# yuhang1008/WildGS-SLAM-Blackwell

Measured on AMD Instinct MI355X. Metric: rasterised Gaussians/s fwd+bwd @1M pts 1080p; PSNR vs ref, higher is better.
Workload: dtype f32; 1 GPU; configs[2]: 1000000 Gaussians, 1920x1080, SH3, single-view fwd+bwd, pose grad on; gaussians=1000000, image=1920x1080, sh_degree=3, num_rendered=13015374, parallelism=dp1 (keyframe views), dp_exchange=none

## Files before the change

wildgs-slam-blackwell_amd/csrc/capi.hip:

```cpp
#include <cstdarg>
#include <cstdio>
#include <cstdlib>
#include <cstring>
#include <vector>

#include <immintrin.h>

#include "wgsr.h"
#include "wgsr_common.h"
#include "wgsr_internal.h"

namespace wgsr {

namespace {
thread_local char g_err[1024] = "";

struct HostCounters {
  uint32_t* buf = nullptr;
  hipEvent_t ev = nullptr;
  hipStream_t side = nullptr;
  hipEvent_t pre = nullptr;
  uint4* mbox = nullptr;
  uint32_t seq = 0;
};
constexpr int kMaxDevices = 64;
int device_slot() {
  int dev = 0;
  return hipGetDevice(&dev) == hipSuccess && dev >= 0 && dev < kMaxDevices ? dev : -1;
}
struct BinningGuess {
  int P = -1, W = 0, H = 0, bshift = -1;
  size_t bytes = 0;
};
BinningGuess& binning_guess() {
  thread_local BinningGuess g[kMaxDevices];
  const int dev = device_slot();
  return g[dev < 0 ? 0 : dev];
}

bool publish_counts() {
  static const bool on = [] {
    const char* e = getenv("WGSR_PUBLISH_COUNTS");
    return !(e && e[0] == '0');
  }();
  return on;
}

HostCounters& host_counters() {
  thread_local HostCounters per_dev[kMaxDevices];
  const int dev = device_slot();
  HostCounters& hc = per_dev[dev < 0 ? 0 : dev];
  if (!hc.buf) {
    void* p = nullptr;
    if (hipHostMalloc(&p, kCounterBytes, hipHostMallocDefault) != hipSuccess) p = nullptr;
    hc.buf = static_cast<uint32_t*>(p);
    if (hipEventCreateWithFlags(&hc.ev, hipEventDisableTiming) != hipSuccess) hc.ev = nullptr;
    if (hipStreamCreateWithFlags(&hc.side, hipStreamNonBlocking) != hipSuccess) hc.side = nullptr;
    if (hc.side && hipEventCreateWithFlags(&hc.pre, hipEventDisableTiming) != hipSuccess) hc.pre = nullptr;
    if (!hc.pre) hc.side = nullptr;
    void* m = nullptr;
    if (publish_counts() &&
        hipHostMalloc(&m, 256, hipHostMallocCoherent | hipHostMallocMapped) == hipSuccess) {
      hc.mbox = static_cast<uint4*>(m);
      *hc.mbox = make_uint4(0u, 0u, 0u, 0u);
    }
  }
  return hc;
}

struct DevCounters {
  uint32_t* buf = nullptr;
  int parity = 0;
  bool failed = false;
};
DevCounters* dev_counters(hipStream_t s) {
  thread_local DevCounters per_dev[kMaxDevices];
  const int dev = device_slot();
// ... 174 lines not shown
  BinLayout BL;
  size_t lists_bytes, bds_bytes, total;
  BinningPlan(size_t N_rect, size_t N_bin, int bshift, bool bin_depth)
      : BL(N_rect), lists_bytes(bshift ? align256(4 * (N_bin << (2 * bshift))) : 0),
        bds_bytes(bin_depth ? align256(16 * N_bin) : 0), total(BL.total + lists_bytes + bds_bytes) {}
};

struct Counts {
  size_t N_rect, N, N_bin;
  uint32_t flags;
  bool published;
};

int start_counts_readback(const Fwd& f, bool bin_depth, HostCounters& hc, PublishJob* pub) {
  if (!hc.buf || !hc.ev) return set_error(WGSR_EHIP, "pinned counter buffer / event allocation failed");
  if (bin_depth && hc.mbox) {
    *pub = PublishJob{f.counter, hc.mbox, hc.seq = (hc.seq % 0xFFFFFFu) + 1u};
  } else if (hc.side && !bin_depth) {
    HIPCHK(hipEventRecord(hc.pre, f.s));
    HIPCHK(hipStreamWaitEvent(hc.side, hc.pre, 0));
    HIPCHK(hipMemcpyAsync(hc.buf, f.counter, kCounterBytes, hipMemcpyDeviceToHost, hc.side));
    HIPCHK(hipEventRecord(hc.ev, hc.side));
  } else {
    HIPCHK(hipMemcpyAsync(hc.buf, f.counter, kCounterBytes, hipMemcpyDeviceToHost, f.s));
    HIPCHK(hipEventRecord(hc.ev, f.s));
  }
  return WGSR_OK;
}

int wait_counts(const Fwd& f, HostCounters& hc, const PublishJob& pub, Counts* c) {
  if (!pub.counter) {
    HIPCHK(hipEventSynchronize(hc.ev));
  } else {
    uint4 rec = make_uint4(0u, 0u, 0u, 0u);
    auto poll = [&]() {
      asm volatile("" ::: "memory");
      const __m128i v = _mm_load_si128(reinterpret_cast<const __m128i*>(const_cast<const uint4*>(hc.mbox)));
      _mm_storeu_si128(reinterpret_cast<__m128i*>(&rec), v);
      return (rec.x >> 8) == pub.seq;
    };
    uint32_t polls = 0;
    while (!poll()) {
      _mm_pause();
      if ((++polls & 1023u) == 0) {
        const hipError_t q = hipStreamQuery(f.s);
        if (q == hipErrorNotReady) continue;
        HIPCHK(q);
        bool seen = false;
        for (int k = 0; k < (1 << 16) && !(seen = poll()); ++k) _mm_pause();
        if (seen) break;
        hc.mbox = nullptr;
        break;
      }
    }
    if (hc.mbox && !(rec.x & 0x80u)) {
      *c = Counts{rec.y, rec.z, rec.w, rec.x & 0x7Fu, true};
      return WGSR_OK;
    }
    HIPCHK(hipMemcpyAsync(hc.buf, f.counter, kCounterBytes, hipMemcpyDeviceToHost, f.s));
    HIPCHK(hipStreamSynchronize(f.s));
  }
  *c = Counts{0, 0, 0, hc.buf[1], false};
  const uint64_t* partial = reinterpret_cast<const uint64_t*>(hc.buf + 4);
  for (int i = 0; i < kRectPairLanes; ++i) {
    c->N_rect += partial[i];
    c->N += partial[kRectPairLanes + i];
    c->N_bin += partial[2 * kRectPairLanes + i];
  }
  return WGSR_OK;
}

int read_depth_range(const Fwd& f, HostCounters& hc, const Counts& c, uint32_t* hi, uint32_t* nlo) {
  if (c.published) {
    HIPCHK(hipMemcpyAsync(hc.buf, f.counter, kCounterBytes, hipMemcpyDeviceToHost, f.s));
    HIPCHK(hipStreamSynchronize(f.s));
  }
  const uint32_t* rw = hc.buf + kDepthRangeOffset / 4;
  *hi = *nlo = 0;
  for (int i = 0; i < kRectPairLanes; ++i) {
    *hi = rw[i] > *hi ? rw[i] : *hi;
    *nlo = rw[kRectPairLanes + i] > *nlo ? rw[kRectPairLanes + i] : *nlo;
  }
  return WGSR_OK;
}

ZeroJob preprocess_zero_job(const Fwd& f, const DevCounters* dc, DepthSched sched) {
  const size_t P = (size_t)f.a.P;
  ZeroJob zj{};
  auto add = [&](void* p, size_t words) {
    if (words) { zj.p[zj.count] = static_cast<float*>(p); zj.n[zj.count++] = words; }
  };
  if (dc) add(dc->buf + (size_t)(dc->parity ^ 1) * (kCounterBytes / 4), kCounterBytes / 4);
  size_t sup_off = depth_sort_sup_offset_words(P);
  const size_t sup_words = sched == DepthSched::kFull     ? sort_sup_words(P, 0, kDepthBits, &sup_off)
                           : sched == DepthSched::kGlobal ? depth_sort_sup_words(P)
                                                          : 0;
  add(f.g<uint32_t>(f.GL.hist) + sup_off, sup_words);
// ... 6 lines not shown
  const size_t P = (size_t)f.a.P;
  uint32_t *dkey = f.g<uint32_t>(GL.dkey), *dkey_alt = f.g<uint32_t>(GL.dkey_alt), *dval = f.g<uint32_t>(GL.dval),
           *dval_alt = f.g<uint32_t>(GL.dval_alt), *hist = f.g<uint32_t>(GL.hist);
  StageTimer T(kStDepthSort, f.s);
  if (full) {
    const bool sup_zeroed = sort_sup_words(P, 0, kDepthBits, nullptr) != 0;
    bool in_alt = false;
    STAGE(f.a, f.s, radix_sort_pairs(dkey, dkey_alt, dval, dval_alt, true, P, 0, kDepthBits, hist,
                                     f.g<uint32_t>(GL.totals), f.s, &in_alt, nullptr, nullptr, sup_zeroed));
    if (in_alt != kFullDepthInAlt) return set_error(WGSR_EHIP, "internal: depth sort parity");
    *depth_order = kFullDepthInAlt ? dval_alt : dval;
    return WGSR_OK;
  }
  if (zero_sup)
    HIPCHK(hipMemsetAsync(hist + depth_sort_sup_offset_words(P), 0, 4 * depth_sort_sup_words(P), f.s));
  STAGE(f.a, f.s, launch_depth_sort(dkey, dkey_alt, dval, dval_alt, P, f.counter + kDepthRangeOffset / 4,
                                    f.counter + 2, hist, f.s));
  *depth_order = dval_alt;
  return WGSR_OK;
}

int queue_scan(const Fwd& f, const uint32_t* depth_order, const PublishJob& pj) {
  const GeomLayout& GL = f.GL;
  StageTimer T(kStOffsetsScan, f.s);
  if (f.bshift) {
    STAGE(f.a, f.s, packed_scan_blocks(f.g<uint32_t>(GL.tb), 1, depth_order, (size_t)f.a.P, f.g<uint32_t>(GL.bsum),
                                       f.s, f.g<uint2>(GL.bsup), pj));
  } else {
    STAGE(f.a, f.s, exclusive_scan_gather(&f.g<ListRec>(GL.lrec)->w.w, depth_order, (size_t)f.a.P,
                                          f.g<uint32_t>(GL.offs), f.g<uint32_t>(GL.slot_start),
                                          f.g<uint32_t>(GL.bsum), f.g<uint32_t>(GL.counter), f.s,
// ... 150 lines not shown
  }
  Fwd f{a, s, Grid(a), GeomLayout((size_t)a.P), ImageLayout(a.W, a.H), bin_shift(a), out_color, out_depth, out_opacity,
        n_touched};
  if (int e = f.alloc(geom_alloc, image_alloc, ctx)) return e;
  DevCounters* dc = dev_counters(s);
  f.counter = dc ? dc->buf + (size_t)dc->parity * (kCounterBytes / 4) : at<uint32_t>(f.geom, f.GL.counter);
  if (!dc) HIPCHK(hipMemsetAsync(f.counter, 0, kCounterBytes, s));
  const DepthSched sched = depth_schedule(f.bshift);
  struct SyncOnError {
    hipStream_t s;
    bool armed = false;
    ~SyncOnError() { if (armed) (void)hipStreamSynchronize(s); }
  } sync_on_error{s};
  { StageTimer T(kStPreprocess, s);
  const hipError_t pe = launch_preprocess(a, f.geom, radii, n_touched, f.counter + 1,
                                          reinterpret_cast<unsigned long long*>(f.counter + 4), f.bshift,
                                          preprocess_zero_job(f, dc, sched), s, f.im<uint32_t>(f.IL.meta));
  if (pe == hipSuccess && dc) dc->parity ^= 1;
  sync_on_error.armed = true;
  STAGE(a, s, pe); }

  HostCounters& hc = host_counters();
  PublishJob pub{};
  if (int e = start_counts_readback(f, sched == DepthSched::kBins, hc, &pub)) return e;
  const uint32_t* depth_order = nullptr;
  if (sched != DepthSched::kBins)
    if (int e = queue_depth_sort(f, sched == DepthSched::kFull, false, &depth_order)) return e;
  if (int e = queue_scan(f, depth_order, pub)) return e;
  BinningGuess& bg = binning_guess();
  void* binning = nullptr;
  size_t binning_have = 0;
  if (bg.P == a.P && bg.W == a.W && bg.H == a.H && bg.bshift == f.bshift && bg.bytes > 0) {
    binning_have = bg.bytes + bg.bytes / 16;
    binning = call_alloc(binning_alloc, ctx, binning_have);
    if (!binning) binning_have = 0;
  }
  Counts c;
  if (int e = wait_counts(f, hc, pub, &c)) return e;
  sync_on_error.armed = false;

  const bool bins_too_full = sched == DepthSched::kBins &&
                             c.N_bin > bin_depth_max_avg() * (size_t)Bins(f.grid.gx, f.grid.gy, f.bshift).n;
  if (bins_too_full) {
// ... 66 lines not shown
  if (!f.bshift || depth_schedule(f.bshift) != DepthSched::kBins)
    return set_error(WGSR_EINVAL, "capacity mode needs sort bins with the per-bin depth sort");
  if (!((size_t)8 << sort_bits(Bins(f.grid.gx, f.grid.gy, f.bshift).n) <= (size_t)16 * f.grid.nt))
    return set_error(WGSR_EINVAL, "capacity mode: the bin bounds do not fit the tile_m region");
  if (int e = f.alloc(geom_alloc, image_alloc, ctx)) return e;
  const size_t C = (size_t)cap;
  const BinningPlan plan(C, C, f.bshift, true);
  void* binning = call_alloc(binning_alloc, ctx, plan.total);
  if (!binning) return set_error(WGSR_EALLOC, "binning buffer allocation failed");
  f.counter = at<uint32_t>(f.geom, f.GL.counter);
  uint32_t* meta = at<uint32_t>(f.image, f.IL.meta);
  HIPCHK(launch_zero_u32(f.counter, kCounterBytes / 4, s));
  const ZeroJob zj = preprocess_zero_job(f, nullptr, DepthSched::kBins);
  { StageTimer T(kStPreprocess, s);
  STAGE(a, s, launch_preprocess(a, f.geom, radii, n_touched, f.counter + 1,
                                reinterpret_cast<unsigned long long*>(f.counter + 4), f.bshift, zj, s, meta)); }
  STAGE(a, s, launch_cap_counts(reinterpret_cast<const unsigned long long*>(f.counter + 4), (uint64_t)C, (uint64_t)C,
                                counts, meta, s));
  if (int e = queue_scan(f, nullptr, PublishJob{})) return e;
  g_depth_order_off = -1;
  return queue_lists_and_render(f, binning, plan, nullptr, true, C, counts + 4);
}

}

namespace wgsr {
namespace {
int render_backward_pairs(const wgsr_raster_args& a, const void* geom, void* binning, void* image,
                          int64_t num_rendered, const float* dL_dcolor, const float* dL_ddepth,
                          wgsr_alloc_fn scratch_alloc, void* ctx, const ZeroJob& zero, hipStream_t s,
                          float4** partial_out, uint8_t** pflag_out) {
  if (!geom || !image || (num_rendered > 0 && !binning))
    return set_error(WGSR_EINVAL, "missing forward state buffers");
  const Grid grid(a);
// ... 150 lines not shown
```

wildgs-slam-blackwell_amd/csrc/raster_pre.hip:

```cpp
#include <algorithm>

#include "raster_sh.h"
#include "wgsr_common.h"
#include "wgsr_internal.h"

namespace wgsr {

namespace {

__device__ __forceinline__ f3 sh_to_rgb(int deg, const float* sh, f3 dir, uint32_t& clamp_bits) {
#pragma clang fp contract(off)
  auto term = [](float c, const float* v) -> f3 { return {c * v[0], c * v[1], c * v[2]}; };
  auto plus = [](f3 a, f3 b) -> f3 { return {a.x + b.x, a.y + b.y, a.z + b.z}; };
  auto minus = [](f3 a, f3 b) -> f3 { return {a.x - b.x, a.y - b.y, a.z - b.z}; };
  f3 r = term(SH_C0, sh);
  if (deg > 0) {
    const float x = dir.x, y = dir.y, z = dir.z;
    r = minus(plus(minus(r, term(SH_C1 * y, sh + 3)), term(SH_C1 * z, sh + 6)), term(SH_C1 * x, sh + 9));
    if (deg > 1) {
      const float xx = x * x, yy = y * y, zz = z * z, xy = x * y, yz = y * z, xz = x * z;
      r = plus(r, term(SH_C2[0] * xy, sh + 12));
      r = plus(r, term(SH_C2[1] * yz, sh + 15));
      r = plus(r, term(SH_C2[2] * (2.f * zz - xx - yy), sh + 18));
      r = plus(r, term(SH_C2[3] * xz, sh + 21));
// ... 89 lines not shown
      tab.y |= len << (8 * (k - 4));
      tab.w |= (uint32_t)(xa - x0) << (8 * (k - 4));
    }
    cnt += len;
  }
  lrec[i].tab = tab;
  if (!finish) clamped[i] = 0u;
  const uint32_t nb = cnt == 0 ? 0u
                               : (uint32_t)((((x1 - 1) >> bshift) - (x0 >> bshift) + 1) *
                                            (((y1 - 1) >> bshift) - (y0 >> bshift) + 1));
  w = make_uint4((uint32_t)r, cnt, cnt | (nb << 16), __float_as_uint(pv.z));
  return make_uint3((uint32_t)((x1 - x0) * (y1 - y0)), cnt, nb);
}

__device__ __forceinline__ void wave_pair_counts(const uint3 ac, uint32_t khi, uint32_t knlo,
                                                 unsigned long long* __restrict__ rect_pairs,
                                                 unsigned long long* __restrict__ list_pairs,
                                                 unsigned long long* __restrict__ bin_pairs,
                                                 uint32_t* __restrict__ drange) {
  const uint32_t slot = blockIdx.x % kRectPairLanes;
  unsigned long long area, cnt, nbin;
  if (wave_any(ac.x >= (1u << 26))) {
    area = ac.x;
    cnt = ac.y;
    nbin = ac.z;
#pragma unroll
    for (int off = 32; off >= 1; off >>= 1) {
      area += __shfl_xor(area, off, 64);
      cnt += __shfl_xor(cnt, off, 64);
      nbin += __shfl_xor(nbin, off, 64);
    }
  } else {
    area = wave_total_u32(ac.x);
    cnt = wave_total_u32(ac.y);
    nbin = wave_total_u32(ac.z);
  }
  const uint32_t kh = wave_maximum_u32(khi), kn = wave_maximum_u32(knlo);
  if (threadIdx.x % 64 == 0) {
    atomicAdd(&rect_pairs[slot], area);
    atomicAdd(&list_pairs[slot], cnt);
    atomicAdd(&bin_pairs[slot], nbin);
    if (kh) atomicMax(&drange[slot], kh);
    if (kn) atomicMax(&drange[kRectPairLanes + slot], kn);
  }
}

constexpr int kPreWave = 64;

template <int kD, int kCh>
__device__ __forceinline__ f3 sh_rgb_lds(const float* __restrict__ s_sh, int lane, f3 dir, uint32_t& cbits) {
  constexpr int K = (kD + 1) * (kD + 1), NF = 3 * K, NCH = (NF + kCh - 1) / kCh;
  float sh[NCH * kCh];
#pragma unroll
  for (int k = 0; k < NCH; ++k) {
    if constexpr (kCh >= 4) {
      const float4 v = reinterpret_cast<const float4*>(s_sh)[k * 64 + lane];
      sh[4 * k] = v.x;
      sh[4 * k + 1] = v.y;
// ... 3 lines not shown
      sh[k] = s_sh[k * 64 + lane];
    }
  }
  return sh_to_rgb(kD, sh, dir, cbits);
}

template <int kCh, int kD>
__global__ __launch_bounds__(kPreWave) void k_preprocess2(
    int P, int D, int M, const float* __restrict__ means, const float* __restrict__ scales,
    const float* __restrict__ rots, const float* __restrict__ opac, const float* __restrict__ shs,
    const float* __restrict__ colors, const float* __restrict__ cov_pre, float scale_mod,
    const float* __restrict__ viewm, const float* __restrict__ projm, const float* __restrict__ campos_p, int W,
    int H, float tanx, float tany, int gx, int gy, int prefiltered, float4* __restrict__ splat,
    ListRec* __restrict__ lrec, uint32_t* __restrict__ clamped,
    uint32_t* __restrict__ dkey, int32_t* __restrict__ radii, int32_t* __restrict__ n_touched,
    uint32_t* __restrict__ err_flag, unsigned long long* __restrict__ rect_pairs,
    unsigned long long* __restrict__ list_pairs, unsigned long long* __restrict__ bin_pairs, int bshift,
    uint32_t* __restrict__ tb, uint8_t* __restrict__ gflag, uint32_t* __restrict__ drange, const ZeroJob zero,
    uint32_t* __restrict__ meta) {
  extern __shared__ float s_sh[];
  const int lane = threadIdx.x;
  const int i0 = blockIdx.x * kPreWave, i = i0 + lane;
  constexpr bool sh_on = kD >= 0;
  const int ic = min(i, P - 1);
  const int ir = cov_pre ? 0 : ic;
  const float* __restrict__ sp = cov_pre ? cov_pre : scales;
  const float* __restrict__ rp = cov_pre ? cov_pre : rots;
  const f3 pl = mk3(means[3 * ic], means[3 * ic + 1], means[3 * ic + 2]);
  const f3 sl = mk3(sp[3 * ir], sp[3 * ir + 1], sp[3 * ir + 2]);
  const float4 ql = make_float4(rp[4 * ir], rp[4 * ir + 1], rp[4 * ir + 2], rp[4 * ir + 3]);
  const float ol = opac[ic];
  asm volatile("" ::"v"(pl.x), "v"(pl.y), "v"(pl.z), "v"(sl.x), "v"(sl.y), "v"(sl.z), "v"(ql.x), "v"(ql.y),
               "v"(ql.z), "v"(ql.w), "v"(ol));
  auto load_slab = [&]() {
// ... 38 lines not shown
    __builtin_amdgcn_s_waitcnt(0);
    __syncthreads();
    if (i < P && w.x != 0u) {
#pragma clang fp contract(off)
      f3 dir = sub3(p, mk3(campos_p[0], campos_p[1], campos_p[2]));
      const float len = sqrtf(dot3(dir, dir));
      dir = mk3(dir.x / len, dir.y / len, dir.z / len);
      uint32_t cbits = 0;
      const f3 rgb = sh_rgb_lds<(kD < 0 ? 0 : kD), kCh>(s_sh, lane, dir, cbits);
      splat[3 * (size_t)i + 0] = ab[0];
      splat[3 * (size_t)i + 1] = ab[1];
      splat[3 * (size_t)i + 2] = make_float4(rgb.x, rgb.y, rgb.z, __uint_as_float(w.w));
      clamped[i] = cbits;
    }
  }
  wave_pair_counts(ac, khi, knlo, rect_pairs, list_pairs, bin_pairs, drange);
  zero_share(zero, blockIdx.x, gridDim.x, lane, kPreWave);
  if (blockIdx.x == 0 && lane == 0) {
    meta[1] = 0u;
    meta[2] = 0u;
  }
}

__global__ __launch_bounds__(256) void k_mark_visible(int P, const float* __restrict__ means,
                                                      const float* __restrict__ viewm, uint8_t* __restrict__ present) {
  const int i = blockIdx.x * blockDim.x + threadIdx.x;
  if (i >= P) return;
  const f3 p = mk3(means[3 * i], means[3 * i + 1], means[3 * i + 2]);
  const f3 pv = xform43(viewm, p);
  present[i] = pv.z > kNearZ ? 1 : 0;
}

}


__global__ __launch_bounds__(64) void k_cap_counts(const unsigned long long* __restrict__ partial,
                                                   uint64_t cap_rect, uint64_t cap_bin, uint32_t* __restrict__ counts,
                                                   uint32_t* __restrict__ meta) {
  const int t = threadIdx.x;
  unsigned long long r = partial[t], e = partial[kRectPairLanes + t], b = partial[2 * kRectPairLanes + t];
#pragma unroll
  for (int off = 32; off >= 1; off >>= 1) {
    r += __shfl_xor(r, off, 64);
    e += __shfl_xor(e, off, 64);
    b += __shfl_xor(b, off, 64);
  }
  if (t == 0) {
    const uint32_t ovf = (r > cap_rect || b > cap_bin) ? 1u : 0u;
    counts[0] = (uint32_t)min(r, 0xFFFFFFFFull);
    counts[1] = (uint32_t)min(e, 0xFFFFFFFFull);
    counts[2] = (uint32_t)min(b, 0xFFFFFFFFull);
    counts[3] = ovf;
    counts[4] = (uint32_t)min(b, (unsigned long long)cap_bin);
    meta[1] = ovf;
  }
}
static_assert(kRectPairLanes == 64, "k_cap_counts: one lane per partial");

hipError_t launch_cap_counts(const unsigned long long* partial, uint64_t cap_rect, uint64_t cap_bin, uint32_t* counts,
                             uint32_t* meta, hipStream_t s) {
  hipLaunchKernelGGL(k_cap_counts, dim3(1), dim3(64), 0, s, partial, cap_rect, cap_bin, counts, meta);
  return hipGetLastError();
}

hipError_t launch_preprocess(const wgsr_raster_args& a, void* geom, int32_t* radii, int32_t* n_touched,
                             uint32_t* err_flag, unsigned long long* rect_pairs, int bshift, const ZeroJob& zero,
                             hipStream_t s, uint32_t* meta) {
  unsigned long long* list_pairs = rect_pairs + kRectPairLanes;
  unsigned long long* bin_pairs = rect_pairs + 2 * kRectPairLanes;
  uint32_t* drange = reinterpret_cast<uint32_t*>(rect_pairs + 3 * kRectPairLanes);
  if (a.P == 0) return hipSuccess;
  const GeomLayout L(a.P);
  const int gx = (a.W + kTile - 1) / kTile, gy = (a.H + kTile - 1) / kTile;
  const bool sh_on = a.shs && !a.colors;
  const bool ch4 = sh_on && (a.M * 3) % 4 == 0 && (reinterpret_cast<uintptr_t>(a.shs) & 15) == 0;
  const int nf = 3 * (a.D + 1) * (a.D + 1);
  const int kch = ch4 ? 4 : 1;
  const size_t lds2 = sh_on ? sizeof(float) * 64 * (size_t)(((nf + kch - 1) / kch) * kch) : 0;
  using PreKernel = decltype(&k_preprocess2<1, -1>);
  static constexpr PreKernel kPre[2][4] = {{k_preprocess2<1, 0>, k_preprocess2<1, 1>, k_preprocess2<1, 2>,
                                            k_preprocess2<1, 3>},
                                           {k_preprocess2<4, 0>, k_preprocess2<4, 1>, k_preprocess2<4, 2>,
                                            k_preprocess2<4, 3>}};
  const PreKernel kern = sh_on ? kPre[ch4 ? 1 : 0][std::min(std::max(a.D, 0), 3)] : k_preprocess2<1, -1>;
  hipLaunchKernelGGL(kern, dim3((a.P + kPreWave - 1) / kPreWave), dim3(kPreWave),
                     lds2, s, a.P, a.D, a.M, a.means3D, a.scales, a.rotations, a.opacities, a.shs, a.colors,
                     a.cov3D_precomp, a.scale_modifier, a.viewmatrix, a.projmatrix, a.campos, a.W, a.H, a.tan_fovx,
                     a.tan_fovy, gx, gy, a.prefiltered, at<float4>(geom, L.splat), at<ListRec>(geom, L.lrec),
                     at<uint32_t>(geom, L.clamped), at<uint32_t>(geom, L.dkey), radii, n_touched, err_flag, rect_pairs,
                     list_pairs, bin_pairs, bshift, at<uint32_t>(geom, L.tb), at<uint8_t>(geom, L.gflag), drange, zero,
                     meta);
  return hipGetLastError();
}

hipError_t launch_mark_visible(int P, const float* means3D, const float* view, uint8_t* present, hipStream_t s) {
  if (P == 0) return hipSuccess;
  hipLaunchKernelGGL(k_mark_visible, dim3((P + 255) / 256), dim3(256), 0, s, P, means3D, view, present);
  return hipGetLastError();
}

}
```

wildgs-slam-blackwell_amd/csrc/sort.hip:

```cpp
#include <stdlib.h>
#include <string.h>

#include "wgsr_common.h"
#include "wgsr_internal.h"

namespace wgsr {

namespace {

__device__ __forceinline__ uint32_t block_excl_scan256(uint32_t v, uint32_t* s_tmp4, uint32_t* total) {
  const int t = threadIdx.x, w = t >> 6, lane = t & 63;
  uint32_t inc = wave_incl_scan(v);
  if (lane == 63) s_tmp4[w] = inc;
  __syncthreads();
  uint32_t base = 0, tot = 0;
#pragma unroll
  for (int i = 0; i < 4; ++i) {
    uint32_t x = s_tmp4[i];
    base += (i < w) ? x : 0u;
    tot += x;
  }
  __syncthreads();
  if (total) *total = tot;
  return base + inc - v;
// ... 332 lines not shown
  __syncthreads();
  const uint32_t cnt = (size_t)n > blk0 ? (uint32_t)min((size_t)kT, (size_t)n - blk0) : 0u;
#pragma unroll
  for (int r = 0; r < K; ++r) {
    const uint32_t i = (uint32_t)t + (uint32_t)NT * r;
    if (i < cnt) {
      const uint2 kv = s_buf[i];
      const uint32_t d = (kv.x >> shift) & mask;
      const uint32_t dst = s_gbase[d] + (i - s_lbase[d]);
      kout[dst] = kv.x;
      vout[dst] = kv.y;
    }
  }
}

static_assert(kRectPairLanes == 64, "one range word per lane");
__device__ __forceinline__ int bitlen32(uint32_t x) {
  return x ? 32 - __clz((int)x) : 0;
}
__device__ __forceinline__ uint32_t wave_max_u32_uniform(uint32_t x) {
  x = max(x, (uint32_t)__builtin_amdgcn_update_dpp(0, (int)x, 0xB1, 0xf, 0xf, true));
  x = max(x, (uint32_t)__builtin_amdgcn_update_dpp(0, (int)x, 0x4E, 0xf, 0xf, true));
  x = max(x, (uint32_t)__builtin_amdgcn_update_dpp(0, (int)x, 0x114, 0xf, 0xf, true));
  x = max(x, (uint32_t)__builtin_amdgcn_update_dpp(0, (int)x, 0x118, 0xf, 0xf, true));
  const uint32_t a = (uint32_t)__builtin_amdgcn_readlane((int)x, 15), b = (uint32_t)__builtin_amdgcn_readlane((int)x, 31);
  const uint32_t c = (uint32_t)__builtin_amdgcn_readlane((int)x, 47), d = (uint32_t)__builtin_amdgcn_readlane((int)x, 63);
  return max(max(a, b), max(c, d));
}
__device__ __forceinline__ uint2 depth_range_reduce(const uint32_t* __restrict__ range) {
  const int lane = threadIdx.x & 63;
  return make_uint2(wave_max_u32_uniform(range[lane]), wave_max_u32_uniform(range[kRectPairLanes + lane]));
}
__device__ __forceinline__ DepthKeyPlan depth_plan_from2(const uint32_t* __restrict__ range2) {
  return depth_key_plan(range2[0], ~range2[1]);
}

template <int I, int PASS>
__global__ __launch_bounds__(256) void k_depth_hist(const uint32_t* __restrict__ keys, uint32_t n,
                                                    const uint32_t* __restrict__ range, uint32_t* __restrict__ range2,
                                                    uint32_t* __restrict__ hist, uint32_t* __restrict__ sup) {
  __shared__ uint32_t s_h[kDepthMaxDigits];
  const int t = threadIdx.x;
  uint32_t k[I];
  const int nv = load_run<I>(keys, n, (size_t)blockIdx.x * (256 * I) + (size_t)t * I, k);
#pragma unroll
  for (int q = 0; q < kDepthMaxDigits / 256; ++q) s_h[t + 256 * q] = 0;
  DepthKeyPlan pl;
  if (PASS == 0) {
    const uint2 r = depth_range_reduce(range);
    if (blockIdx.x == 0 && t == 0) {
      range2[0] = r.x;
      range2[1] = r.y;
    }
    pl = depth_key_plan(r.x, ~r.y);
// ... 365 lines not shown
                                              totals, stream, result_in_alt, digit_bounds, bounds_done, sup_zeroed,
                                              ndev, wide_threads);
    case kSmallSortItems:
      return radix_sort_tiled<kSmallSortItems>(keys, keys_alt, vals, vals_alt, vals_iota, n, begin_bit, end_bit,
                                               status, totals, stream, result_in_alt, digit_bounds, bounds_done,
                                               sup_zeroed, ndev, wide_threads);
    default:
      return radix_sort_tiled<kSortItems>(keys, keys_alt, vals, vals_alt, vals_iota, n, begin_bit, end_bit, status,
                                          totals, stream, result_in_alt, digit_bounds, bounds_done, sup_zeroed,
                                          ndev, wide_threads);
  }
}

template <int I>
static hipError_t depth_sort_tiled(uint32_t* keys, uint32_t* keys_alt, uint32_t* vals, uint32_t* vals_alt, size_t n,
                                   const uint32_t* range, uint32_t* range2, uint32_t* scratch, hipStream_t s) {
  const uint32_t nb = (uint32_t)((n + 256 * I - 1) / (256 * I)), nsup = (nb + kSupBlocks - 1) / kSupBlocks;
  uint32_t* hist = scratch;
  uint32_t* sup = scratch + depth_sort_sup_offset_words(n);
  const size_t sup_pass = (size_t)kDepthMaxDigits * nsup;
  const uint32_t un = (uint32_t)n;
  hipLaunchKernelGGL((k_depth_hist<I, 0>), dim3(nb), dim3(256), 0, s, keys, un, range, range2, hist, sup);
  hipLaunchKernelGGL((k_depth_scatter<I, 0>), dim3(nb), dim3(256), 0, s, keys, vals, un, range2, hist, sup, nsup,
                     keys_alt, vals_alt);
  hipLaunchKernelGGL((k_depth_hist<I, 1>), dim3(nb), dim3(256), 0, s, keys_alt, un, range, range2, hist,
                     sup + sup_pass);
  hipLaunchKernelGGL((k_depth_scatter<I, 1>), dim3(nb), dim3(256), 0, s, keys_alt, vals_alt, un, range2, hist,
                     sup + sup_pass, nsup, keys, vals);
  hipLaunchKernelGGL((k_depth_hist<I, 2>), dim3(nb), dim3(256), 0, s, keys, un, range, range2, hist,
                     sup + 2 * sup_pass);
  hipLaunchKernelGGL((k_depth_scatter<I, 2>), dim3(nb), dim3(256), 0, s, keys, vals, un, range2, hist,
                     sup + 2 * sup_pass, nsup, keys_alt, vals_alt);
  return hipGetLastError();
}

hipError_t launch_depth_sort(uint32_t* keys, uint32_t* keys_alt, uint32_t* vals, uint32_t* vals_alt, size_t n,
                             const uint32_t* range, uint32_t* range2, uint32_t* scratch, hipStream_t s) {
  if (n == 0) return hipSuccess;
  if (n > (size_t)kStCount) return hipErrorInvalidValue;
  switch (sort_items(n)) {
    case kTinySortItems:
      return depth_sort_tiled<kTinySortItems>(keys, keys_alt, vals, vals_alt, n, range, range2, scratch, s);
    case kSmallSortItems:
      return depth_sort_tiled<kSmallSortItems>(keys, keys_alt, vals, vals_alt, n, range, range2, scratch, s);
    default:
      return depth_sort_tiled<kSortItems>(keys, keys_alt, vals, vals_alt, n, range, range2, scratch, s);
  }
}

hipError_t exclusive_scan_gather(const uint32_t* vals, const uint32_t* idx, size_t n, uint32_t* out,
                                 uint32_t* scatter_out, uint32_t* bsum, uint32_t* total_out, hipStream_t stream,
                                 uint32_t stride) {
// ... 25 lines not shown
```

wildgs-slam-blackwell_amd/csrc/wgsr_common.h:

```cpp
#pragma once

#include <hip/hip_runtime.h>
#include <stdint.h>

namespace wgsr {

constexpr int kTile = 16;
constexpr int kWave = 64;
constexpr float kNearZ = 0.2f;
constexpr float kMinAlpha = 1.0f / 255.0f;
constexpr float kMaxAlpha = 0.99f;
constexpr float kMinT = 0.0001f;
constexpr float kL2E = 1.4426950408889634f;
constexpr float kConicSq = -0.5f * kL2E;
constexpr float kConicXY = -kL2E;
constexpr float kUnConicSq = -2.0f / kL2E, kUnConicXY = -1.0f / kL2E;

typedef float v2f __attribute__((ext_vector_type(2)));

__device__ __forceinline__ int lane_id() { return __lane_id(); }

__device__ __forceinline__ uint32_t lanes_below(uint64_t mask) {
  return __builtin_amdgcn_mbcnt_hi((uint32_t)(mask >> 32),
                                   __builtin_amdgcn_mbcnt_lo((uint32_t)mask, 0u));
// ... 533 lines not shown
constexpr int kTinySortItems = 4;
constexpr int kSortItems = 16;
constexpr int kWideSortThreads = 512;
constexpr size_t kSmallSortN = size_t(1) << 21;
constexpr size_t kTinySortN = size_t(1) << 18;
constexpr int kScanTile = 1024;
constexpr int kPackedScanTile = 256;

__host__ __device__ inline int sort_items(size_t n) {
  return n <= kTinySortN ? kTinySortItems : (n <= kSmallSortN ? kSmallSortItems : kSortItems);
}
__host__ __device__ inline uint32_t sort_blocks(size_t n) {
  const size_t tile = 256 * (size_t)sort_items(n);
  return (uint32_t)((n + tile - 1) / tile);
}
constexpr int kRectPairLanes = 64;
constexpr size_t kDepthRangeOffset = 16 + 3 * 8 * kRectPairLanes;
constexpr size_t kCounterBytes = kDepthRangeOffset + 2 * 4 * kRectPairLanes;

struct PublishJob {
  const uint32_t* counter = nullptr;
  uint4* host = nullptr;
  uint32_t seq = 0;
};
__device__ __forceinline__ void publish_counts(const PublishJob& pj, int lane) {
  const unsigned long long* partial = reinterpret_cast<const unsigned long long*>(pj.counter + 4);
  unsigned long long v[3];
#pragma unroll
  for (int k = 0; k < 3; ++k) {
    v[k] = partial[k * kRectPairLanes + lane];
#pragma unroll
    for (int off = 32; off >= 1; off >>= 1) v[k] += (unsigned long long)__shfl_xor((long long)v[k], off, 64);
  }
  if (lane == 0) {
    const bool big = ((v[0] | v[1] | v[2]) >> 32) != 0;
    *pj.host = make_uint4((pj.seq << 8) | (pj.counter[1] & 0x7Fu) | (big ? 0x80u : 0u), (uint32_t)v[0],
                          (uint32_t)v[1], (uint32_t)v[2]);
  }
}
static_assert(kRectPairLanes == 64, "publish_counts: one lane per partial");

constexpr int kDepthPasses = 3;
constexpr int kDepthMaxDigitBits = 10;
constexpr int kDepthMaxDigits = 1 << kDepthMaxDigitBits;
struct DepthKeyPlan {
  uint32_t lo_r, cul;
  int R;
  int shift[kDepthPasses], bits[kDepthPasses];
  int extra_shift, extra_bits;
};
__host__ __device__ inline DepthKeyPlan depth_key_plan(uint32_t hi, uint32_t lo) {
  DepthKeyPlan p;
  if (hi < lo) {
    p.lo_r = 0u;
    p.cul = 0u;
// ... 141 lines not shown
```

wildgs-slam-blackwell_amd/csrc/wgsr_internal.h:

```cpp
#pragma once

#include <hip/hip_runtime.h>
#include <stdint.h>

#include "wgsr.h"

namespace wgsr {

int radix_passes(int begin_bit, int end_bit);
hipError_t radix_sort_pairs(uint32_t* keys, uint32_t* keys_alt, uint32_t* vals, uint32_t* vals_alt, bool vals_iota,
                            size_t n, int begin_bit, int end_bit, uint32_t* status, uint32_t* totals,
                            hipStream_t stream, bool* result_in_alt,
                            uint2* digit_bounds = nullptr, bool* bounds_done = nullptr, bool sup_zeroed = false,
                            const uint32_t* ndev = nullptr, int wide_threads = 0);
size_t sort_sup_words(size_t n, int begin_bit, int end_bit, size_t* offset_words);

hipError_t launch_depth_sort(uint32_t* keys, uint32_t* keys_alt, uint32_t* vals, uint32_t* vals_alt, size_t n,
                             const uint32_t* range, uint32_t* range2, uint32_t* scratch, hipStream_t s);

hipError_t exclusive_scan_gather(const uint32_t* vals, const uint32_t* idx, size_t n, uint32_t* out,
                                 uint32_t* scatter_out, uint32_t* bsum, uint32_t* total_out, hipStream_t stream,
                                 uint32_t stride = 1);

hipError_t packed_scan_blocks(const uint32_t* packed, uint32_t stride, const uint32_t* idx, size_t n, void* bsum,
                              hipStream_t stream, void* bsup, const PublishJob& pub = PublishJob{});

int num_bits(uint32_t n);

int set_error(int code, const char* fmt, ...);

hipError_t launch_preprocess(const wgsr_raster_args& a, void* geom, int32_t* radii, int32_t* n_touched,
                             uint32_t* err_flag, unsigned long long* rect_pairs, int bshift, const ZeroJob& zero, hipStream_t s, uint32_t* meta);
hipError_t launch_cap_counts(const unsigned long long* partial, uint64_t cap_rect, uint64_t cap_bin, uint32_t* counts,
                             uint32_t* meta, hipStream_t s);
hipError_t launch_mark_visible(int P, const float* means3D, const float* view, uint8_t* present, hipStream_t s);

hipError_t launch_duplicate_bins(const wgsr_raster_args& a, void* geom, const uint32_t* depth_order, int bshift,
                                 uint8_t* pflag, uint32_t* keys, uint32_t* vals, const ZeroJob& zero,
                                 uint32_t* meta, hipStream_t s, uint32_t cap_slots = 0xFFFFFFFFu,
                                 uint32_t cap_pairs = 0xFFFFFFFFu);
hipError_t launch_duplicate(const wgsr_raster_args& a, const void* geom, const uint32_t* sorted_g, uint32_t P,
                            uint32_t* keys, uint32_t* slot_g, uint8_t* pflag, hipStream_t s);
hipError_t make_bin_bounds(const uint32_t* sorted_keys, uint32_t NB, int nbins, uint2* bounds, bool bounds_done,
                           hipStream_t s);
hipError_t launch_expand_bins(const wgsr_raster_args& a, const uint32_t* sorted_keys, const uint32_t* sorted_g,
                              uint32_t NB, int bshift, uint2* bounds, bool bounds_done, uint32_t* lists, uint2* ranges,
                              uint32_t* tile_len, uint32_t* meta, hipStream_t s);
hipError_t launch_ranges(const uint32_t* sorted_keys, uint32_t N, int ntiles, uint2* ranges, uint32_t* len,
// ... 41 lines not shown
```

Baseline: 1.466 billion Gaussians/s.

## Spread preprocess counters over 256 cache-line slots and read back totals header

```diff
diff --git a/wildgs-slam-blackwell_amd/csrc/capi.hip b/wildgs-slam-blackwell_amd/csrc/capi.hip
--- a/wildgs-slam-blackwell_amd/csrc/capi.hip
+++ b/wildgs-slam-blackwell_amd/csrc/capi.hip
@@ -17,6 +17,7 @@
 
 struct HostCounters {
   uint32_t* buf = nullptr;
+  bool whole = false;
   hipEvent_t ev = nullptr;
   hipStream_t side = nullptr;
   hipEvent_t pre = nullptr;
@@ -39,11 +40,8 @@
 }
 
 bool publish_counts() {
-  static const bool on = [] {
-    const char* e = getenv("WGSR_PUBLISH_COUNTS");
-    return !(e && e[0] == '0');
-  }();
-  return on;
+  const char* e = getenv("WGSR_PUBLISH_COUNTS");
+  return !(e && e[0] == '0');
 }
 
 HostCounters& host_counters() {
@@ -59,8 +57,7 @@
     if (hc.side && hipEventCreateWithFlags(&hc.pre, hipEventDisableTiming) != hipSuccess) hc.pre = nullptr;
     if (!hc.pre) hc.side = nullptr;
     void* m = nullptr;
-    if (publish_counts() &&
-        hipHostMalloc(&m, 256, hipHostMallocCoherent | hipHostMallocMapped) == hipSuccess) {
+    if (hipHostMalloc(&m, 256, hipHostMallocCoherent | hipHostMallocMapped) == hipSuccess) {
       hc.mbox = static_cast<uint4*>(m);
       *hc.mbox = make_uint4(0u, 0u, 0u, 0u);
     }
@@ -265,22 +262,53 @@
 
 int start_counts_readback(const Fwd& f, bool bin_depth, HostCounters& hc, PublishJob* pub) {
   if (!hc.buf || !hc.ev) return set_error(WGSR_EHIP, "pinned counter buffer / event allocation failed");
-  if (bin_depth && hc.mbox) {
-    *pub = PublishJob{f.counter, hc.mbox, hc.seq = (hc.seq % 0xFFFFFFu) + 1u};
-  } else if (hc.side && !bin_depth) {
+  *pub = PublishJob{f.counter, nullptr, 0u};
+  if (bin_depth && hc.mbox && publish_counts()) {
+    pub->host = hc.mbox;
+    pub->seq = hc.seq = (hc.seq % 0xFFFFFFu) + 1u;
+  } else if (bin_depth) {
+  } else if (hc.side) {
     HIPCHK(hipEventRecord(hc.pre, f.s));
     HIPCHK(hipStreamWaitEvent(hc.side, hc.pre, 0));
     HIPCHK(hipMemcpyAsync(hc.buf, f.counter, kCounterBytes, hipMemcpyDeviceToHost, hc.side));
     HIPCHK(hipEventRecord(hc.ev, hc.side));
+    hc.whole = true;
   } else {
     HIPCHK(hipMemcpyAsync(hc.buf, f.counter, kCounterBytes, hipMemcpyDeviceToHost, f.s));
     HIPCHK(hipEventRecord(hc.ev, f.s));
-  }
-  return WGSR_OK;
+    hc.whole = true;
+  }
+  return WGSR_OK;
+}
+
+int copy_counts_header(const Fwd& f, HostCounters& hc, bool record) {
+  HIPCHK(hipMemcpyAsync(hc.buf, f.counter, kCountHeaderBytes, hipMemcpyDeviceToHost, f.s));
+  if (record) HIPCHK(hipEventRecord(hc.ev, f.s));
+  else HIPCHK(hipStreamSynchronize(f.s));
+  hc.whole = false;
+  return WGSR_OK;
+}
+
+CountTotals host_count_totals(const HostCounters& hc) {
+  if (!hc.whole) {
+    CountTotals t;
+    memcpy(&t, hc.buf + kCountTotalsOffset / 4, sizeof t);
+    return t;
+  }
+  CountTotals t{0, 0, 0, 0, 0};
+  const CountSlot* slots = count_slots(hc.buf);
+  for (int i = 0; i < kCountSlots; ++i) {
+    t.rect += slots[i].rect;
+    t.list += slots[i].list;
+    t.bin += slots[i].bin;
+    t.key_hi = slots[i].key_hi > t.key_hi ? slots[i].key_hi : t.key_hi;
+    t.key_nlo = slots[i].key_nlo > t.key_nlo ? slots[i].key_nlo : t.key_nlo;
+  }
+  return t;
 }
 
 int wait_counts(const Fwd& f, HostCounters& hc, const PublishJob& pub, Counts* c) {
-  if (!pub.counter) {
+  if (!pub.host) {
     HIPCHK(hipEventSynchronize(hc.ev));
   } else {
     uint4 rec = make_uint4(0u, 0u, 0u, 0u);
@@ -308,30 +336,19 @@
       *c = Counts{rec.y, rec.z, rec.w, rec.x & 0x7Fu, true};
       return WGSR_OK;
     }
-    HIPCHK(hipMemcpyAsync(hc.buf, f.counter, kCounterBytes, hipMemcpyDeviceToHost, f.s));
-    HIPCHK(hipStreamSynchronize(f.s));
-  }
-  *c = Counts{0, 0, 0, hc.buf[1], false};
-  const uint64_t* partial = reinterpret_cast<const uint64_t*>(hc.buf + 4);
-  for (int i = 0; i < kRectPairLanes; ++i) {
-    c->N_rect += partial[i];
-    c->N += partial[kRectPairLanes + i];
-    c->N_bin += partial[2 * kRectPairLanes + i];
-  }
+    if (int e = copy_counts_header(f, hc, false)) return e;
+  }
+  const CountTotals t = host_count_totals(hc);
+  *c = Counts{(size_t)t.rect, (size_t)t.list, (size_t)t.bin, hc.buf[1], false};
   return WGSR_OK;
 }
 
 int read_depth_range(const Fwd& f, HostCounters& hc, const Counts& c, uint32_t* hi, uint32_t* nlo) {
-  if (c.published) {
-    HIPCHK(hipMemcpyAsync(hc.buf, f.counter, kCounterBytes, hipMemcpyDeviceToHost, f.s));
-    HIPCHK(hipStreamSynchronize(f.s));
-  }
-  const uint32_t* rw = hc.buf + kDepthRangeOffset / 4;
-  *hi = *nlo = 0;
-  for (int i = 0; i < kRectPairLanes; ++i) {
-    *hi = rw[i] > *hi ? rw[i] : *hi;
-    *nlo = rw[kRectPairLanes + i] > *nlo ? rw[kRectPairLanes + i] : *nlo;
-  }
+  if (c.published)
+    if (int e = copy_counts_header(f, hc, false)) return e;
+  const CountTotals t = host_count_totals(hc);
+  *hi = t.key_hi;
+  *nlo = t.key_nlo;
   return WGSR_OK;
 }
 
@@ -368,7 +385,7 @@
   }
   if (zero_sup)
     HIPCHK(hipMemsetAsync(hist + depth_sort_sup_offset_words(P), 0, 4 * depth_sort_sup_words(P), f.s));
-  STAGE(f.a, f.s, launch_depth_sort(dkey, dkey_alt, dval, dval_alt, P, f.counter + kDepthRangeOffset / 4,
+  STAGE(f.a, f.s, launch_depth_sort(dkey, dkey_alt, dval, dval_alt, P, count_slots(f.counter),
                                     f.counter + 2, hist, f.s));
   *depth_order = dval_alt;
   return WGSR_OK;
@@ -549,7 +566,7 @@
   } sync_on_error{s};
   { StageTimer T(kStPreprocess, s);
   const hipError_t pe = launch_preprocess(a, f.geom, radii, n_touched, f.counter + 1,
-                                          reinterpret_cast<unsigned long long*>(f.counter + 4), f.bshift,
+                                          count_slots(f.counter), f.bshift,
                                           preprocess_zero_job(f, dc, sched), s, f.im<uint32_t>(f.IL.meta));
   if (pe == hipSuccess && dc) dc->parity ^= 1;
   sync_on_error.armed = true;
@@ -562,6 +579,8 @@
   if (sched != DepthSched::kBins)
     if (int e = queue_depth_sort(f, sched == DepthSched::kFull, false, &depth_order)) return e;
   if (int e = queue_scan(f, depth_order, pub)) return e;
+  if (sched == DepthSched::kBins && !pub.host)
+    if (int e = copy_counts_header(f, hc, true)) return e;
   BinningGuess& bg = binning_guess();
   void* binning = nullptr;
   size_t binning_have = 0;
@@ -658,10 +677,10 @@
   const ZeroJob zj = preprocess_zero_job(f, nullptr, DepthSched::kBins);
   { StageTimer T(kStPreprocess, s);
   STAGE(a, s, launch_preprocess(a, f.geom, radii, n_touched, f.counter + 1,
-                                reinterpret_cast<unsigned long long*>(f.counter + 4), f.bshift, zj, s, meta)); }
-  STAGE(a, s, launch_cap_counts(reinterpret_cast<const unsigned long long*>(f.counter + 4), (uint64_t)C, (uint64_t)C,
+                                count_slots(f.counter), f.bshift, zj, s, meta)); }
+  STAGE(a, s, launch_cap_counts(count_slots(f.counter), (uint64_t)C, (uint64_t)C,
                                 counts, meta, s));
-  if (int e = queue_scan(f, nullptr, PublishJob{})) return e;
+  if (int e = queue_scan(f, nullptr, PublishJob{f.counter, nullptr, 0u})) return e;
   g_depth_order_off = -1;
   return queue_lists_and_render(f, binning, plan, nullptr, true, C, counts + 4);
 }
diff --git a/wildgs-slam-blackwell_amd/csrc/raster_pre.hip b/wildgs-slam-blackwell_amd/csrc/raster_pre.hip
--- a/wildgs-slam-blackwell_amd/csrc/raster_pre.hip
+++ b/wildgs-slam-blackwell_amd/csrc/raster_pre.hip
@@ -127,11 +127,8 @@
 }
 
 __device__ __forceinline__ void wave_pair_counts(const uint3 ac, uint32_t khi, uint32_t knlo,
-                                                 unsigned long long* __restrict__ rect_pairs,
-                                                 unsigned long long* __restrict__ list_pairs,
-                                                 unsigned long long* __restrict__ bin_pairs,
-                                                 uint32_t* __restrict__ drange) {
-  const uint32_t slot = blockIdx.x % kRectPairLanes;
+                                                 CountSlot* __restrict__ slots) {
+  CountSlot* __restrict__ rec = slots + blockIdx.x % kCountSlots;
   unsigned long long area, cnt, nbin;
   if (wave_any(ac.x >= (1u << 26))) {
     area = ac.x;
@@ -150,11 +147,11 @@
   }
   const uint32_t kh = wave_maximum_u32(khi), kn = wave_maximum_u32(knlo);
   if (threadIdx.x % 64 == 0) {
-    atomicAdd(&rect_pairs[slot], area);
-    atomicAdd(&list_pairs[slot], cnt);
-    atomicAdd(&bin_pairs[slot], nbin);
-    if (kh) atomicMax(&drange[slot], kh);
-    if (kn) atomicMax(&drange[kRectPairLanes + slot], kn);
+    atomicAdd(&rec->rect, area);
+    atomicAdd(&rec->list, cnt);
+    atomicAdd(&rec->bin, nbin);
+    if (kh) atomicMax(&rec->key_hi, kh);
+    if (kn) atomicMax(&rec->key_nlo, kn);
   }
 }
 
@@ -188,10 +185,8 @@
     int H, float tanx, float tany, int gx, int gy, int prefiltered, float4* __restrict__ splat,
     ListRec* __restrict__ lrec, uint32_t* __restrict__ clamped,
     uint32_t* __restrict__ dkey, int32_t* __restrict__ radii, int32_t* __restrict__ n_touched,
-    uint32_t* __restrict__ err_flag, unsigned long long* __restrict__ rect_pairs,
-    unsigned long long* __restrict__ list_pairs, unsigned long long* __restrict__ bin_pairs, int bshift,
-    uint32_t* __restrict__ tb, uint8_t* __restrict__ gflag, uint32_t* __restrict__ drange, const ZeroJob zero,
-    uint32_t* __restrict__ meta) {
+    uint32_t* __restrict__ err_flag, CountSlot* __restrict__ slots, int bshift,
+    uint32_t* __restrict__ tb, uint8_t* __restrict__ gflag, const ZeroJob zero, uint32_t* __restrict__ meta) {
   extern __shared__ float s_sh[];
   const int lane = threadIdx.x;
   const int i0 = blockIdx.x * kPreWave, i = i0 + lane;
@@ -260,7 +255,7 @@
       clamped[i] = cbits;
     }
   }
-  wave_pair_counts(ac, khi, knlo, rect_pairs, list_pairs, bin_pairs, drange);
+  wave_pair_counts(ac, khi, knlo, slots);
   zero_share(zero, blockIdx.x, gridDim.x, lane, kPreWave);
   if (blockIdx.x == 0 && lane == 0) {
     meta[1] = 0u;
@@ -280,17 +275,12 @@
 }
 
 
-__global__ __launch_bounds__(64) void k_cap_counts(const unsigned long long* __restrict__ partial,
+__global__ __launch_bounds__(64) void k_cap_counts(const CountSlot* __restrict__ slots,
                                                    uint64_t cap_rect, uint64_t cap_bin, uint32_t* __restrict__ counts,
                                                    uint32_t* __restrict__ meta) {
   const int t = threadIdx.x;
-  unsigned long long r = partial[t], e = partial[kRectPairLanes + t], b = partial[2 * kRectPairLanes + t];
-#pragma unroll
-  for (int off = 32; off >= 1; off >>= 1) {
-    r += __shfl_xor(r, off, 64);
-    e += __shfl_xor(e, off, 64);
-    b += __shfl_xor(b, off, 64);
-  }
+  const CountTotals tot = count_slots_reduce(slots, t);
+  const unsigned long long r = tot.rect, e = tot.list, b = tot.bin;
   if (t == 0) {
     const uint32_t ovf = (r > cap_rect || b > cap_bin) ? 1u : 0u;
     counts[0] = (uint32_t)min(r, 0xFFFFFFFFull);
@@ -301,20 +291,16 @@
     meta[1] = ovf;
   }
 }
-static_assert(kRectPairLanes == 64, "k_cap_counts: one lane per partial");
-
-hipError_t launch_cap_counts(const unsigned long long* partial, uint64_t cap_rect, uint64_t cap_bin, uint32_t* counts,
+
+hipError_t launch_cap_counts(const CountSlot* slots, uint64_t cap_rect, uint64_t cap_bin, uint32_t* counts,
                              uint32_t* meta, hipStream_t s) {
-  hipLaunchKernelGGL(k_cap_counts, dim3(1), dim3(64), 0, s, partial, cap_rect, cap_bin, counts, meta);
+  hipLaunchKernelGGL(k_cap_counts, dim3(1), dim3(64), 0, s, slots, cap_rect, cap_bin, counts, meta);
   return hipGetLastError();
 }
 
 hipError_t launch_preprocess(const wgsr_raster_args& a, void* geom, int32_t* radii, int32_t* n_touched,
-                             uint32_t* err_flag, unsigned long long* rect_pairs, int bshift, const ZeroJob& zero,
+                             uint32_t* err_flag, CountSlot* slots, int bshift, const ZeroJob& zero,
                              hipStream_t s, uint32_t* meta) {
-  unsigned long long* list_pairs = rect_pairs + kRectPairLanes;
-  unsigned long long* bin_pairs = rect_pairs + 2 * kRectPairLanes;
-  uint32_t* drange = reinterpret_cast<uint32_t*>(rect_pairs + 3 * kRectPairLanes);
   if (a.P == 0) return hipSuccess;
   const GeomLayout L(a.P);
   const int gx = (a.W + kTile - 1) / kTile, gy = (a.H + kTile - 1) / kTile;
@@ -333,9 +319,8 @@
                      lds2, s, a.P, a.D, a.M, a.means3D, a.scales, a.rotations, a.opacities, a.shs, a.colors,
                      a.cov3D_precomp, a.scale_modifier, a.viewmatrix, a.projmatrix, a.campos, a.W, a.H, a.tan_fovx,
                      a.tan_fovy, gx, gy, a.prefiltered, at<float4>(geom, L.splat), at<ListRec>(geom, L.lrec),
-                     at<uint32_t>(geom, L.clamped), at<uint32_t>(geom, L.dkey), radii, n_touched, err_flag, rect_pairs,
-                     list_pairs, bin_pairs, bshift, at<uint32_t>(geom, L.tb), at<uint8_t>(geom, L.gflag), drange, zero,
-                     meta);
+                     at<uint32_t>(geom, L.clamped), at<uint32_t>(geom, L.dkey), radii, n_touched, err_flag, slots,
+                     bshift, at<uint32_t>(geom, L.tb), at<uint8_t>(geom, L.gflag), zero, meta);
   return hipGetLastError();
 }
 
diff --git a/wildgs-slam-blackwell_amd/csrc/sort.hip b/wildgs-slam-blackwell_amd/csrc/sort.hip
--- a/wildgs-slam-blackwell_amd/csrc/sort.hip
+++ b/wildgs-slam-blackwell_amd/csrc/sort.hip
@@ -370,7 +370,6 @@
   }
 }
 
-static_assert(kRectPairLanes == 64, "one range word per lane");
 __device__ __forceinline__ int bitlen32(uint32_t x) {
   return x ? 32 - __clz((int)x) : 0;
 }
@@ -383,9 +382,17 @@
   const uint32_t c = (uint32_t)__builtin_amdgcn_readlane((int)x, 47), d = (uint32_t)__builtin_amdgcn_readlane((int)x, 63);
   return max(max(a, b), max(c, d));
 }
-__device__ __forceinline__ uint2 depth_range_reduce(const uint32_t* __restrict__ range) {
+static_assert(kCountSlots % 64 == 0, "depth_range_reduce: whole rounds of 64 lanes");
+__device__ __forceinline__ uint2 depth_range_reduce(const CountSlot* __restrict__ range) {
   const int lane = threadIdx.x & 63;
-  return make_uint2(wave_max_u32_uniform(range[lane]), wave_max_u32_uniform(range[kRectPairLanes + lane]));
+  constexpr int R = kCountSlots / 64;
+  uint2 k[R];
+#pragma unroll
+  for (int r = 0; r < R; ++r) k[r] = *reinterpret_cast<const uint2*>(&range[64 * r + lane].key_hi);
+  uint2 m = k[0];
+#pragma unroll
+  for (int r = 1; r < R; ++r) m = make_uint2(max(m.x, k[r].x), max(m.y, k[r].y));
+  return make_uint2(wave_max_u32_uniform(m.x), wave_max_u32_uniform(m.y));
 }
 __device__ __forceinline__ DepthKeyPlan depth_plan_from2(const uint32_t* __restrict__ range2) {
   return depth_key_plan(range2[0], ~range2[1]);
@@ -393,7 +400,7 @@
 
 template <int I, int PASS>
 __global__ __launch_bounds__(256) void k_depth_hist(const uint32_t* __restrict__ keys, uint32_t n,
-                                                    const uint32_t* __restrict__ range, uint32_t* __restrict__ range2,
+                                                    const CountSlot* __restrict__ range, uint32_t* __restrict__ range2,
                                                     uint32_t* __restrict__ hist, uint32_t* __restrict__ sup) {
   __shared__ uint32_t s_h[kDepthMaxDigits];
   const int t = threadIdx.x;
@@ -789,7 +796,7 @@
 
 template <int I>
 static hipError_t depth_sort_tiled(uint32_t* keys, uint32_t* keys_alt, uint32_t* vals, uint32_t* vals_alt, size_t n,
-                                   const uint32_t* range, uint32_t* range2, uint32_t* scratch, hipStream_t s) {
+                                   const CountSlot* range, uint32_t* range2, uint32_t* scratch, hipStream_t s) {
   const uint32_t nb = (uint32_t)((n + 256 * I - 1) / (256 * I)), nsup = (nb + kSupBlocks - 1) / kSupBlocks;
   uint32_t* hist = scratch;
   uint32_t* sup = scratch + depth_sort_sup_offset_words(n);
@@ -810,7 +817,7 @@
 }
 
 hipError_t launch_depth_sort(uint32_t* keys, uint32_t* keys_alt, uint32_t* vals, uint32_t* vals_alt, size_t n,
-                             const uint32_t* range, uint32_t* range2, uint32_t* scratch, hipStream_t s) {
+                             const CountSlot* range, uint32_t* range2, uint32_t* scratch, hipStream_t s) {
   if (n == 0) return hipSuccess;
   if (n > (size_t)kStCount) return hipErrorInvalidValue;
   switch (sort_items(n)) {
diff --git a/wildgs-slam-blackwell_amd/csrc/wgsr_common.h b/wildgs-slam-blackwell_amd/csrc/wgsr_common.h
--- a/wildgs-slam-blackwell_amd/csrc/wgsr_common.h
+++ b/wildgs-slam-blackwell_amd/csrc/wgsr_common.h
@@ -571,31 +571,77 @@
   const size_t tile = 256 * (size_t)sort_items(n);
   return (uint32_t)((n + tile - 1) / tile);
 }
-constexpr int kRectPairLanes = 64;
-constexpr size_t kDepthRangeOffset = 16 + 3 * 8 * kRectPairLanes;
-constexpr size_t kCounterBytes = kDepthRangeOffset + 2 * 4 * kRectPairLanes;
+constexpr int kCountSlots = 256;
+struct alignas(64) CountSlot {
+  unsigned long long rect, list, bin;
+  uint32_t key_hi, key_nlo;
+  uint32_t pad[8];
+};
+static_assert(sizeof(CountSlot) == 64, "one 64-byte segment per slot");
+struct CountTotals {
+  unsigned long long rect, list, bin;
+  uint32_t key_hi, key_nlo;
+};
+constexpr size_t kCountTotalsOffset = 16;
+constexpr size_t kCountHeaderBytes = 64;
+constexpr size_t kCountSlotsOffset = kCountHeaderBytes;
+constexpr size_t kCounterBytes = kCountSlotsOffset + sizeof(CountSlot) * kCountSlots;
+static_assert(kCountTotalsOffset + sizeof(CountTotals) <= kCountHeaderBytes, "the totals fit the header");
+__host__ __device__ inline CountSlot* count_slots(uint32_t* counter) {
+  return reinterpret_cast<CountSlot*>(counter + kCountSlotsOffset / 4);
+}
+__host__ __device__ inline const CountSlot* count_slots(const uint32_t* counter) {
+  return reinterpret_cast<const CountSlot*>(counter + kCountSlotsOffset / 4);
+}
+
+static_assert(kCountSlots % 64 == 0, "count_slots_reduce: whole rounds of 64 lanes");
+__device__ __forceinline__ CountTotals count_slots_reduce(const CountSlot* __restrict__ slots, int lane) {
+  constexpr int R = kCountSlots / 64;
+  uint4 a[R], b[R];
+#pragma unroll
+  for (int r = 0; r < R; ++r) {
+    const uint4* p = reinterpret_cast<const uint4*>(slots + 64 * r + lane);
+    a[r] = p[0];
+    b[r] = p[1];
+  }
+  unsigned long long v[3] = {0ull, 0ull, 0ull};
+  uint32_t hi = 0u, nlo = 0u;
+#pragma unroll
+  for (int r = 0; r < R; ++r) {
+    v[0] += (unsigned long long)a[r].x | ((unsigned long long)a[r].y << 32);
+    v[1] += (unsigned long long)a[r].z | ((unsigned long long)a[r].w << 32);
+    v[2] += (unsigned long long)b[r].x | ((unsigned long long)b[r].y << 32);
+    hi = max(hi, b[r].z);
+    nlo = max(nlo, b[r].w);
+  }
+#pragma unroll
+  for (int off = 32; off >= 1; off >>= 1) {
+#pragma unroll
+    for (int k = 0; k < 3; ++k) v[k] += (unsigned long long)__shfl_xor((long long)v[k], off, 64);
+    hi = max(hi, (uint32_t)__shfl_xor((int)hi, off, 64));
+    nlo = max(nlo, (uint32_t)__shfl_xor((int)nlo, off, 64));
+  }
+  return CountTotals{v[0], v[1], v[2], hi, nlo};
+}
 
 struct PublishJob {
-  const uint32_t* counter = nullptr;
+  uint32_t* counter = nullptr;
   uint4* host = nullptr;
   uint32_t seq = 0;
 };
 __device__ __forceinline__ void publish_counts(const PublishJob& pj, int lane) {
-  const unsigned long long* partial = reinterpret_cast<const unsigned long long*>(pj.counter + 4);
-  unsigned long long v[3];
-#pragma unroll
-  for (int k = 0; k < 3; ++k) {
-    v[k] = partial[k * kRectPairLanes + lane];
-#pragma unroll
-    for (int off = 32; off >= 1; off >>= 1) v[k] += (unsigned long long)__shfl_xor((long long)v[k], off, 64);
-  }
+  const CountTotals t = count_slots_reduce(count_slots(pj.counter), lane);
   if (lane == 0) {
-    const bool big = ((v[0] | v[1] | v[2]) >> 32) != 0;
-    *pj.host = make_uint4((pj.seq << 8) | (pj.counter[1] & 0x7Fu) | (big ? 0x80u : 0u), (uint32_t)v[0],
-                          (uint32_t)v[1], (uint32_t)v[2]);
-  }
-}
-static_assert(kRectPairLanes == 64, "publish_counts: one lane per partial");
+    uint4* h = reinterpret_cast<uint4*>(pj.counter + kCountTotalsOffset / 4);
+    h[0] = make_uint4((uint32_t)t.rect, (uint32_t)(t.rect >> 32), (uint32_t)t.list, (uint32_t)(t.list >> 32));
+    h[1] = make_uint4((uint32_t)t.bin, (uint32_t)(t.bin >> 32), t.key_hi, t.key_nlo);
+    if (pj.host) {
+      const bool big = ((t.rect | t.list | t.bin) >> 32) != 0;
+      *pj.host = make_uint4((pj.seq << 8) | (pj.counter[1] & 0x7Fu) | (big ? 0x80u : 0u), (uint32_t)t.rect,
+                            (uint32_t)t.list, (uint32_t)t.bin);
+    }
+  }
+}
 
 constexpr int kDepthPasses = 3;
 constexpr int kDepthMaxDigitBits = 10;
diff --git a/wildgs-slam-blackwell_amd/csrc/wgsr_internal.h b/wildgs-slam-blackwell_amd/csrc/wgsr_internal.h
--- a/wildgs-slam-blackwell_amd/csrc/wgsr_internal.h
+++ b/wildgs-slam-blackwell_amd/csrc/wgsr_internal.h
@@ -16,7 +16,7 @@
 size_t sort_sup_words(size_t n, int begin_bit, int end_bit, size_t* offset_words);
 
 hipError_t launch_depth_sort(uint32_t* keys, uint32_t* keys_alt, uint32_t* vals, uint32_t* vals_alt, size_t n,
-                             const uint32_t* range, uint32_t* range2, uint32_t* scratch, hipStream_t s);
+                             const CountSlot* range, uint32_t* range2, uint32_t* scratch, hipStream_t s);
 
 hipError_t exclusive_scan_gather(const uint32_t* vals, const uint32_t* idx, size_t n, uint32_t* out,
                                  uint32_t* scatter_out, uint32_t* bsum, uint32_t* total_out, hipStream_t stream,
@@ -30,8 +30,8 @@
 int set_error(int code, const char* fmt, ...);
 
 hipError_t launch_preprocess(const wgsr_raster_args& a, void* geom, int32_t* radii, int32_t* n_touched,
-                             uint32_t* err_flag, unsigned long long* rect_pairs, int bshift, const ZeroJob& zero, hipStream_t s, uint32_t* meta);
-hipError_t launch_cap_counts(const unsigned long long* partial, uint64_t cap_rect, uint64_t cap_bin, uint32_t* counts,
+                             uint32_t* err_flag, CountSlot* slots, int bshift, const ZeroJob& zero, hipStream_t s, uint32_t* meta);
+hipError_t launch_cap_counts(const CountSlot* slots, uint64_t cap_rect, uint64_t cap_bin, uint32_t* counts,
                              uint32_t* meta, hipStream_t s);
 hipError_t launch_mark_visible(int P, const float* means3D, const float* view, uint8_t* present, hipStream_t s);
 
```

New measurement: 1.491 billion Gaussians/s (median of 6 runs). 1.7% higher.
